# tomer196/GaUDI

Hardware: AMD Instinct MI355X
Metric: guided molecules/sec (1000-step) (higher is better)
Workload: dtype f32

## Files before the change

gaudi_amd/csrc/gaudi_hip.hip:

```cpp
#include <hip/hip_runtime.h>

#include <algorithm>
#include <climits>
#include <queue>
#include <cmath>
#include <cstdio>
#include <cstdlib>
#include <chrono>
#include <cstring>
#include <map>
#include <mutex>
#include <string>
#include <vector>

#include "../../include/gaudi_hip.h"
#include "sampler_kernel.h"

using namespace gaudi;

struct DevBuf {
  void* p = nullptr;
  size_t cap = 0;
  hipError_t reserve(size_t bytes) {
    if (bytes <= cap) return hipSuccess;
// ... 682 lines not shown
#define X(name) kernel_fn gaudi_kern8s_##name(int hpe, int hpp);
GAUDI_KERNEL8S_TUS(X)
#undef X
static kernel_fn pick_kernel8s(int hpe, int hpp) {
  kernel_fn f = nullptr;
#define X(name) \
  if (!f) f = gaudi_kern8s_##name(hpe, hpp);
  GAUDI_KERNEL8S_TUS(X)
#undef X
  return f;
}

#ifdef GAUDI_STAMP_STUBS
#define GAUDI_KERNEL8S2_TUS(X)
#else
#define GAUDI_KERNEL8S2_TUS(X) X(edm_192) X(fused_tiny) X(fused_192_208)
#endif
#define X(name) kernel_fn gaudi_kern8s2_##name(int hpe, int hpp);
GAUDI_KERNEL8S2_TUS(X)
#undef X
static kernel_fn pick_kernel8s2(int hpe, int hpp) {
  kernel_fn f = nullptr;
#define X(name) \
  if (!f) f = gaudi_kern8s2_##name(hpe, hpp);
  GAUDI_KERNEL8S2_TUS(X)
#undef X
  (void)hpe; (void)hpp;
  return f;
}

#ifdef GAUDI_STAMP_STUBS
// ... 93 lines not shown
  size_t net = 0;
  if (hpe)
    net = std::max(net, (size_t)((gn ? 0 : 4 * N * (hpe + 4)) + kWaves * 16 * (hpe + 4) + 8 * N + kWaves * EW * 9 + (6 + ef) * hpe +
                                 (ef > 2 ? kWaves * EW * ef : 0)));
  if (hpp) net = std::max(net, (size_t)((gn ? 0 : 5 * N * (hpp + 4)) + kWaves * 16 * (hpp + 4) + 12 * N + kWaves * EW * 10 + 32 + 10 * hpp));
  return sizeof(float) * (common_floats(N, D, EW) + net);
}
static size_t gnode_floats(int hpe, int hpp, int N) {
  return std::max((size_t)(hpe ? 4 * N * (hpe + 4) : 0), (size_t)(hpp ? 5 * N * (hpp + 4) : 0));
}

static size_t lds_floats8_base(int hpe, int hpp, int N, int D, int S, int split, int gn = 0) {
  size_t net = 0;
  const int pbuf = gn == 3 ? 4 : 5;
  if (gn == 3) gn = 0;
  if (hpe) net = std::max(net, (size_t)((gn ? w8::gn_lds_buffers(gn) : 5) * N * (hpe + 4) + w8::edge_ring_floats(hpe, split) + 8 * N + 2 * align4(N) + 96 + S * 9 + 8 * hpe));
  if (hpp) net = std::max(net, (size_t)(w8::edge_ring_floats(hpp, split) + (gn ? w8::gn_lds_buffers(gn) : pbuf) * N * (hpp + 4) + 12 * N + 2 * align4(N) + 96 + S * 10 + 32 + 10 * hpp));
  return common_floats8(N, D, S) + net;
}
static size_t gnode_floats8(int hpe, int hpp, int N) {
  return std::max((size_t)(hpe ? 5 * N * (hpe + 4) : 0), (size_t)(hpp ? 5 * N * (hpp + 4) : 0));
}
static bool gn8_stage_fits(int hpe, int hpp, int N) {
  for (int hp : {hpe, hpp})
    if (hp && 2 * (size_t)w8::stage_stride(N * (hp + 4)) > w8::edge_ring_floats(hp, 1)) return false;
  return true;
}
static bool node_f16_fits(int hp, int N, int split, bool gn) {
  if (!hp || !split || !GAUDI_NODE_F16) return true;
  if (N > (gn ? 48 : 32)) return false;
  const int nct = N <= 16 ? 1 : N <= 32 ? 2 : 3;
  const int ring = w8::edge_ring_floats(hp, split);
// ... 16 lines not shown
  const int nch = (T + pub_ch - 1) / pub_ch;
  pub_ch = (T + nch - 1) / nch;
  pubx = (int)std::max(0LL, (long long)S * (16 * pub_ch + 4) - own);
  return true;
}
static size_t lds_bytes8(int hpe, int hpp, int N, int D, int S, int pubx, int split, int gn = 0) {
  return sizeof(float) * (lds_floats8_base(hpe, hpp, N, D, S, split, gn) + (hpp ? pubx : 0));
}

static int launch(gaudi_handle* h, const KParams& P, int hpe, int hpp, long long steps) {
  const bool v8 = h->run_variant == 8;
  const bool se = hpe && h->ecfg.sin_embedding;
  kernel_fn fn = v8   ? (h->run_pg && hpe && hpp ? pick_kernel8mp(hpe, hpp) : h->run_gn8 == 2 ? pick_kernel8gp(hpe, hpp) : h->run_gn8 ? pick_kernel8g(hpe, hpp) : pick_kernel8_mode(hpe, hpp, h->run_split, h->run_mr && hpp))
                 : se ? pick_kernel_se(hpe, hpp, h->run_gn)
                      : h->run_gn ? pick_kernel_g(hpe, hpp) : pick_kernel(hpe, hpp);
  if (v8 && !h->run_gn8 && h->run_split == 1 && !(h->run_mr && hpp) && P.N > 16 && !getenv("GAUDI_NO_FR"))
    if (kernel_fn f2 = pick_kernel8s2(hpe, hpp)) fn = f2;
  if (!fn)
    return fail(h, GAUDI_E_INVALID,
                "no kernel instantiated for padded hidden sizes (" + std::to_string(hpe) + "," + std::to_string(hpp) + ")" +
                    (v8 ? " in the 8-wave family" : se ? " among the sin_embedding kernels" : ""));
  size_t lds = v8 ? lds_bytes8(hpe, hpp, P.N, 3 + P.F, P.EW, P.pubx, h->run_split, h->run_pg && hpe && hpp ? 3 : h->run_gn8)
                  : lds_bytes(hpe, hpp, P.N, 3 + P.F, P.EW, h->run_gn, se ? 24 : 2);
  if (v8 && P.hk_off) lds = sizeof(float) * ((size_t)P.hk_off + (size_t)h->run_hk);
  if (lds > 160 * 1024)
    return fail(h, GAUDI_E_CAPACITY, "molecule needs " + std::to_string(lds) + " B of LDS (>160 KiB): N too large");
  {
    static std::mutex attr_mu;
    static std::map<std::pair<int, const void*>, int> granted_by_fn;
    std::lock_guard<std::mutex> lock(attr_mu);
    int& granted = granted_by_fn[{h->device, (const void*)fn}];
    if ((int)lds > granted) {
// ... 1511 lines not shown
```

gaudi_amd/csrc/w8_edm.h:

```cpp
#pragma once
#include "edm_device.h"
#include "w8_common.h"
#include "w8_split.h"
#include "w8_nodes_f16.h"

namespace gaudi {
namespace w8 {

__host__ __device__ constexpr int gn_lds_buffers(int gn) { return gn == 2 ? 2 : 0; }
template <int HP, int SP = 0, int GN = 0>
struct NetSmem {
  static constexpr bool kGlobalNodes = GN != 0;
  float *h, *p, *q;
  float *agg, *agg1;
  float* ring;
  float *x, *x0;
  uint32_t *pmax, *qmax;
  float* hsc;
  f4* geo;
  float* d0;
  float* trans;
  float* vec;
  float* hk = nullptr;
  __host__ __device__ static int floats(int N, int S) {
    return (GN ? gn_lds_buffers(GN) : 5) * N * (HP + 4) + EdgeRing<HP, SP>::kFloats + 8 * N + 2 * align4(N) + 96 + S * 9 + 8 * HP;
  }
  __device__ void carve(float* base, int N, int S, float* gnode = nullptr) {
    constexpr int LD = HP + 4;
    ring = base; base += EdgeRing<HP, SP>::kFloats;
    if (GN) gnode = assume_global(gnode);
    float*& nb = GN ? gnode : base;
    h = nb; nb += N * LD;
    if (GN == 2) {
      p = base; base += N * LD;
      q = base; base += N * LD;
    } else {
      p = nb; nb += N * LD;
      q = nb; nb += N * LD;
    }
    agg = nb; nb += N * LD;
    agg1 = nb; nb += N * LD;
    x = base; base += 4 * N;
    x0 = base; base += 4 * N;
    pmax = (uint32_t*)base; base += align4(N);
    qmax = (uint32_t*)base; base += align4(N);
    hsc = base; base += 96;
    geo = (f4*)base; base += S * 4;
    d0 = base; base += S;
    trans = base; base += S * 4;
    vec = base;
  }
};

template <class SM>
__device__ __forceinline__ void compute_geo(const SM& sm, const MolGraph& mg, float norm_constant, int tid, bool write_d0) {
  for (int slot = tid; slot < mg.ntiles * 16; slot += kThreads) {
    const uint32_t e = mg.edge[slot];
    const int i = ew_i(e), j = ew_j(e);
    const float dx = sm.x[4 * i + 0] - sm.x[4 * j + 0];
    const float dy = sm.x[4 * i + 1] - sm.x[4 * j + 1];
    const float dz = sm.x[4 * i + 2] - sm.x[4 * j + 2];
// ... 97 lines not shown
  float* const xs0 = sm.ring;
  float* const xs1 = sm.ring + stage_stride(N * LD);
  if constexpr (!RI) er_start<HP>(ring, wbe, lay.gcl(0, 0) + 2 * PK, wave, lane);
  typename NodePFSel<HP, NH>::type pf;
  node_prefetch_x<HP, NH, kAheadOne>(pf, wb, wbe, lay.gcl(0, 0), mg.NC, wave, lane, tw);
  auto hctx = [&]() {
    if constexpr (NH) {
      if constexpr (RI) return node_ctx_h<HP>(sm.ring, EdgeRing<HP, SP>::kFloats, mg.NC, W.hinv, tw, sm.hsc);
      else return node_ctx_h<HP>(ring.slot(ring.par ^ 1), EdgeRing<HP, SP>::kFloats / 2, mg.NC, W.hinv, tw, sm.hsc);
    } else {
      return NodeCtxH{1.f, nullptr, nullptr, tw, nullptr};
    }
  };
  const bool keep = NH && sm.hk != nullptr;
  bool h_kept = false;
  constexpr int NV = (7 * HP + 16 + kThreads - 1) / kThreads;
  VecPF<NV> vpf;
  vec_prefetch<NV, kThreads>(vpf, wb, lay.gcl(0, 0) + 6 * PK, 7 * HP + 16, tid);
  STAMP(ST_EDM_IO);

  for (int l = 0; l < W.L; ++l) {
    compute_geo(sm, mg, W.norm_constant, tid, false);
    STAMP(ST_GEO);
    for (int s = 0; s < W.S; ++s) {
      const int G = lay.gcl(l, s);
      const int Wnext_edge = s + 1 < W.S ? lay.gcl(l, s + 1) + 2 * PK : lay.equ(l) + 2 * PK;
      if constexpr (STG) stage_rows(xs0, sm.h, N * LD, wave, lane);
      for (int idx = tid; idx < N * (LD / 4); idx += kThreads) {
        *(f4*)(sm.agg + 4 * idx) = splat(0.f);
        *(f4*)(sm.agg1 + 4 * idx) = splat(0.f);
// ... 41 lines not shown
            const f4 wv = *(const f4*)(wa + 16 * t + 4 * g);
            sdot += m[0] * wv[0] + m[1] * wv[1] + m[2] * wv[2] + m[3] * wv[3];
          }
          float a = 1.f;
          if (W.attention) a = sigmoid_f(reduce_groups(sdot) + ba);
          const float sc = a * tc.mk;
#pragma unroll
          for (int t = 0; t < T; ++t) acc[t] = acc[t] * sc;
          scatter_runs<HP>(acc, tc, sm.agg, sm.agg1, g);
        }
        STAMP(ST_EDGE_EPI);
      }
      __syncthreads();
      STAMP(ST_BARRIER);
      if constexpr (STG) stage_rows(xs0, sm.h, N * LD, wave, lane);
      for (int idx = tid; idx < N * (HP / 4); idx += kThreads) {
        const int n = idx / (HP / 4), f = 4 * (idx % (HP / 4));
        if constexpr (STG)
          *(f4*)(xs1 + n * LD + f) = (*(const f4*)(sm.agg + n * LD + f) + *(const f4*)(sm.agg1 + n * LD + f)) / W.normf;
        else
          *(f4*)(sm.agg + n * LD + f) = (*(const f4*)(sm.agg + n * LD + f) + *(const f4*)(sm.agg1 + n * LD + f)) / W.normf;
      }
      if constexpr (STG) stage_wait();
      else __syncthreads();
      STAMP(ST_MISC);
      node_gemm_x<HP, EPI_SILU, true, GN, NH, kAheadOne, kAheadOne, FL>(wb, wbe, G + 3 * PK, sm.h, xs0, !h_kept, G + 4 * PK, sm.agg, xs1, bn1, sm.p, nullptr, nullptr,
                                              mg.NC, wave, lane, tw, keep ? node_ctx_keep<HP>(hctx(), sm.hk, mg.NC) : hctx(), pf, G + 5 * PK);
      STAMP(ST_NODE);
      __syncthreads();
      STAMP(ST_BARRIER);
      vec_prefetch<NV, kThreads>(vpf, wb, s + 1 < W.S ? lay.gcl(l, s + 1) + 6 * PK : lay.equ(l) + 3 * PK,
                                 s + 1 < W.S ? 7 * HP + 16 : 5 * HP + 16, tid);
      if constexpr (STG) {
        stage_rows(xs0, sm.p, N * LD, wave, lane);
        stage_wait();
      }
      node_gemm_x<HP, EPI_RESIDUAL_MASK, false, GN, NH, kAheadOne, kAheadOne, FL>(wb, wbe, G + 5 * PK, sm.p, xs0, true, -1, nullptr, nullptr, bn2, sm.h, sm.h, mg.mask,
                                                       mg.NC, wave, lane, tw, hctx(), pf,
                                                       s + 1 < W.S ? lay.gcl(l, s + 1) : lay.equ(l));
      h_kept = false;
      STAMP(ST_NODE);
      __syncthreads();
      STAMP(ST_BARRIER);
    }
    {
      const int E = lay.equ(l);
      const int Wnext_edge = l + 1 < W.L ? lay.gcl(l + 1, 0) + 2 * PK : -1;
      vec_commit<NV, kThreads>(vpf, sm.vec, 5 * HP + 16, tid);
      if (tid < N) {
        sm.pmax[tid] = 0u;
        sm.qmax[tid] = 0u;
      }
      if constexpr (STG) {
        stage_rows(xs0, sm.h, N * LD, wave, lane);
        stage_wait();
// ... 107 lines not shown
```

gaudi_amd/csrc/w8_nodes_f16.h:

```cpp
#pragma once
#include "w8_split.h"

namespace gaudi {
namespace w8 {


constexpr float kLoScale = 2048.f;
#ifndef GAUDI_NODE_ABLATE
#define GAUDI_NODE_ABLATE 0
#endif
constexpr int kAblateH = GAUDI_NODE_ABLATE;
#ifndef GAUDI_NODE_STAMPS
#define GAUDI_NODE_STAMPS 0
#endif
#ifndef GAUDI_NODE_PRIO
#define GAUDI_NODE_PRIO 1
#endif
struct NodeStampH {
  unsigned long long sum[8], last;
  __device__ __forceinline__ void start() { last = __builtin_amdgcn_s_memtime(); }
  __device__ __forceinline__ void mark(int i) {
    const unsigned long long t = __builtin_amdgcn_s_memtime();
    sum[i] += t - last;
    last = t;
// ... 48 lines not shown


__host__ __device__ constexpr int nh_bpos(int c, int g) { return (16 * g + (c ^ g)) * 4; }
struct SplitRowH {
  f4 x;
  uint32_t mx;
};
template <int HP>
__device__ __forceinline__ SplitRowH split_row_load(const float* X, int n, int lane) {
  constexpr int LD = HP + 4;
  SplitRowH r;
  r.x = lane < HP / 4 ? *(const f4*)(X + n * LD + 4 * lane) : splat(0.f);
  r.mx = umax(umax(absbits(r.x[0]), absbits(r.x[1])), umax(absbits(r.x[2]), absbits(r.x[3])));
  return r;
}
template <int HP>
__device__ __forceinline__ void split_row_store(const SplitBufH& sb, const f4 x, uint32_t mx, int n, int lane) {
  constexpr int T = HP / 16, nc = nh_chunks(HP);
  const int m = lane >> 3, g = (lane >> 1) & 3, half = lane & 1;
  int k = 141 - (int)(mx >> 23);
  k = k > 126 ? 126 : k;
  const float s = __builtin_bit_cast(float, (uint32_t)(k + 127) << 23), inv = __builtin_bit_cast(float, (uint32_t)(127 - k) << 23);
  const float y0 = x[0] * s, y1 = x[1] * s, y2 = x[2] * s, y3 = x[3] * s;
  const uint32_t h01 = pk_f16(y0, y1), h23 = pk_f16(y2, y3);
  const f2 f01 = unpk_f16(h01), f23 = unpk_f16(h23);
  const uint32_t l01 = pk_f16((y0 - f01[0]) * kLoScale, (y1 - f01[1]) * kLoScale),
                 l23 = pk_f16((y2 - f23[0]) * kLoScale, (y3 - f23[1]) * kLoScale);
  const int ct = n >> 4, c = n & 15;
  if (m < nc) {
    float* d = sb.chunk(m) + ct * 512 + nh_bpos(c, g) + half * 2;
    *(u2*)d = (u2){h01, h23};
    *(u2*)(d + 256) = (u2){l01, l23};
  } else if (nh_odd(HP) && lane < HP / 4) {
    float* d = sb.tail(HP) + ct * 256 + 4 * (lane - 4 * (T - 1)) * 16 + c;
    d[0] = x[0];
    d[16] = x[1];
    d[32] = x[2];
    d[48] = x[3];
  }
  if (lane == 0) sb.scale(HP)[ct * 16 + c] = inv;
}
template <int HP>
__device__ __forceinline__ void split_rows_h(const SplitBufH& sb, const float* X, int N, int wave, int lane) {
  for (int n = wave; n < N; n += 2 * kWaves) {
    const int n2 = n + kWaves < N ? n + kWaves : n;
    SplitRowH a = split_row_load<HP>(X, n, lane), b = split_row_load<HP>(X, n2, lane);
    a.mx = wave_max_u32(a.mx);
// ... 55 lines not shown
  constexpr int nd = AHEAD < NodeGeoH<HP>::D ? AHEAD : NodeGeoH<HP>::D;
  const TileLanesH<HP> tl(wave, lane);
  static_for<nd>([&](auto d_tag) {
    constexpr int d = decltype(d_tag)::value;
    nh_load<HP>(pf.s[d], wh, 2 * W + d * nh_chunk_floats(HP), wave, tl);
  });
}

struct NodeCtxH {
  float winv;
  float* split_a;
  float* split_b;
  bool ktail;
  float* scales;
  float* scales_b = nullptr;
};

template <int HP, int EPI, bool TWO, int MAXNT, int PIN = kAheadOne, int POUT = kAheadOne, bool FL = false>
__device__ __forceinline__ void node_gemm_h(const WBuf& wh, int Wa, const float* sXa, bool do_split_a, int Wb, const float* sXb,
                                            const float* sBias, float* sY, const float* sRes, const float* sMask, int N, int wave,
                                            int lane, const NodeCtxH& cx, NodePFH<HP>& pf, int nextW = -1, float* gPre = nullptr,
                                            uint32_t* sMaxOut = nullptr ,
                                            NodeStampH* ns = nullptr) {
  (void)ns;
  using G = NodeGeoH<HP>;
  constexpr int T = G::T, LD = HP + 4, NTW = G::NTW, nc = G::nc, D = G::D;
  constexpr int kIn = PIN < D ? PIN : D, kOut = POUT < D ? POUT : D;
  constexpr int kLate = nc < D ? 0 : (GAUDI_NODE_LATE < kOut ? GAUDI_NODE_LATE : kOut);
  const int c = lane & 15, g = lane >> 4;
  const int nt = (MAXNT < 2 || N <= 16) ? 1 : (MAXNT < 3 || N <= 32) ? 2 : 3;
  const bool seq = TWO && cx.split_b == cx.split_a;
  const SplitBufH sa{cx.split_a, nt, cx.scales}, sb{cx.split_b, nt, cx.scales_b != nullptr ? cx.scales_b : cx.scales + kScaleFloatsH};
  const int bpos = nh_bpos(c, g);
// ... 10 lines not shown
    for (int u = 0; u < NTW; ++u) {
      const int t = wave + kWaves * u < T ? wave + kWaves * u : 0;
#pragma unroll
      for (int q = 0; q < 4; ++q) {
        const int ln = (q == 0 || !cx.ktail) ? tl.l[u] : kOOBLane;
        ta[u][q] = __builtin_bit_cast(float, __builtin_amdgcn_raw_buffer_load_b32(wh.r, ln * 4, (2 * Wa + nh_tail_off(HP) + t * 256 + q * 64) * 4, 0));
        if constexpr (TWO)
          tb[u][q] = __builtin_bit_cast(float, __builtin_amdgcn_raw_buffer_load_b32(wh.r, ln * 4, (2 * Wb + nh_tail_off(HP) + t * 256 + q * 64) * 4, 0));
      }
    }
  }
  NSTAMP(0);
  if (!(kAblateH & 1)) {
    const int ls = FL ? fresh(lane) : lane;
    if (do_split_a) split_rows_h<HP>(sa, sXa, N, wave, ls);
    if (TWO && !seq) split_rows_h<HP>(sb, sXb, N, wave, ls);
    NSTAMP(1);
    if (do_split_a || (TWO && !seq)) lds_barrier();
    NSTAMP(2);
  }

  f4 acc0[MAXNT][NTW], acc1[MAXNT][NTW], y[MAXNT][NTW];
#pragma unroll
  for (int j = 0; j < MAXNT; ++j)
#pragma unroll
    for (int u = 0; u < NTW; ++u) {
      const int t = wave + kWaves * u < T ? wave + kWaves * u : 0;
      acc0[j][u] = splat(0.f);
      acc1[j][u] = splat(0.f);
      y[j][u] = sBias != nullptr ? *(const f4*)(sBias + 16 * t + 4 * g) : splat(0.f);
    }
  struct BH {
    u4 h, l;
// ... 92 lines not shown
      lds_barrier();
      split_rows_h<HP>(sb, sXb, N, wave, FL ? fresh(lane) : lane);
      lds_barrier();
    }
    source(std::integral_constant<int, 1>{}, sb);
    late(std::integral_constant<int, kOut - kLate>{});
    fold(sb, tb);
  }
  static_for<D>([&](auto d_tag) {
    if constexpr (decltype(d_tag)::value > kOut - kLate) late(d_tag);
  });
#if GAUDI_NODE_PRIO
  if constexpr (!FL) __builtin_amdgcn_s_setprio(0);
#endif
  const int le = FL ? fresh(lane) : lane, ce = le & 15, ge = le >> 4;
  static_for<MAXNT>([&](auto j_tag) {
    constexpr int j = decltype(j_tag)::value;
    if (j < nt) {
#pragma unroll
      for (int u = 0; u < NTW; ++u) {
        const int t = wave + kWaves * u;
        const int nd = j * 16 + ce;
        f4 yy = y[j][u];
        if (t < T && nd < N) {
          float* dst = sY + nd * LD + 16 * t + 4 * ge;
          const bool pad = G::odd && cx.ktail && t == T - 1 && ge > 0;
          if (pad) yy = splat(0.f);
          if (gPre != nullptr) nstash_store((f4*)(gPre + nd * HP + 16 * t + 4 * ge), yy);
          if (sMaxOut != nullptr) atomicMax(sMaxOut + nd, umax(umax(absbits(yy[0]), absbits(yy[1])), umax(absbits(yy[2]), absbits(yy[3]))));
          if (!pad) {
            if (EPI == EPI_SILU) yy = silu4v(yy);
            if (EPI == EPI_RESIDUAL_MASK) {
              const f4 r = *(const f4*)(sRes + nd * LD + 16 * t + 4 * ge);
              yy = (r + yy) * sMask[nd];
            }
            if (EPI == EPI_MUL_DSILU) {
              const f4 r = *(const f4*)(sRes + nd * LD + 16 * t + 4 * ge);
              yy = yy * dsilu4v(r);
            }
            if (EPI == EPI_ACCUM) yy = *(const f4*)(sRes + nd * LD + 16 * t + 4 * ge) + yy;
          }
          *(f4*)dst = yy;
        }
      }
    }
  });
  NSTAMP(6);
}

#ifndef GAUDI_NODE_F16
#define GAUDI_NODE_F16 1
#endif
template <int SP>
struct NodeMath {
  static constexpr bool kF16 = SP != 0 && GAUDI_NODE_F16 != 0;
};
template <int HP, bool NH>
struct NodePFSel {
  using type = NodePF<HP>;
};
template <int HP>
struct NodePFSel<HP, true> {
  using type = NodePFH<HP>;
};
template <int HP, bool NH, int AHEAD, class PF>
__device__ __forceinline__ void node_prefetch_x(PF& pf, const WBuf& wb, const WBuf& wbe, int W, int N, int wave, int lane, bool tw) {
  if constexpr (NH) node_prefetch_h<HP, AHEAD>(pf, wbe, W, wave, lane);
  else node_prefetch<HP>(pf, wb, W, wave, lane, tw);
}
template <int HP, int EPI, bool TWO, int GN, bool NH, int PIN, int POUT, bool FL = false, class PF>
__device__ __forceinline__ void node_gemm_x(const WBuf& wb, const WBuf& wbe, int Wa, const float* Xa, const float* XaS, bool split_a, int Wb,
                                            const float* Xb, const float* XbS, const float* sBias, float* sY, const float* sRes,
                                            const float* sMask, int N, int wave, int lane, bool tw, const NodeCtxH& cx, PF& pf,
                                            int nextW = -1, float* gPre = nullptr, uint32_t* sMaxOut = nullptr) {
  if constexpr (NH) {
    node_gemm_h<HP, EPI, TWO, GN ? 3 : 2, PIN, POUT, FL>(wbe, Wa, Xa, split_a, Wb, Xb, sBias, sY, sRes, sMask, N, wave, lane, cx, pf, nextW, gPre,
                                                         sMaxOut);
  } else if constexpr (GN != 0) {
    node_gemm_n<HP, EPI, true, 3>(wb, Wa, XaS, Wb, XbS, sBias, sY, sRes, sMask, N, wave, lane, tw, &pf, nextW, gPre);
  } else {
    node_gemm<HP, EPI, true>(wb, Wa, Xa, Wb, Xb, sBias, sY, sRes, sMask, N, wave, lane, tw, &pf, nextW, gPre);
  }
}
__host__ __device__ constexpr bool node_ring_idle(int HP, int SP, bool GN) {
  return GN || (SP != 0 && GAUDI_NODE_F16 != 0 && (SP == 2 || HP < 48));
}
template <int HP>
__device__ __forceinline__ NodeCtxH node_ctx_h(float* region, int cap, int N, float winv, bool ktail, float* scales) {
  const int nct = N <= 16 ? 1 : N <= 32 ? 2 : 3;
  const int need = nh_split_floats(HP, nct);
  return NodeCtxH{winv, region, 2 * need <= cap ? region + need : region, ktail, scales};
}
__host__ __device__ constexpr int nh_keep_floats(int HP, int N) { return nh_split_floats(HP, N <= 16 ? 1 : N <= 32 ? 2 : 3) + kScaleFloatsH; }
template <int HP>
__device__ __forceinline__ NodeCtxH node_ctx_keep(const NodeCtxH& cx, float* keep, int N) {
  const int nct = N <= 16 ? 1 : N <= 32 ? 2 : 3;
  return NodeCtxH{cx.winv, keep + kScaleFloatsH, cx.split_a, cx.ktail, keep, cx.scales};
  (void)nct;
}

}
}
```

gaudi_amd/csrc/w8_pred.h:

```cpp
#pragma once
#include "pred_device.h"
#include "w8_edm.h"

namespace gaudi {
namespace w8 {

template <int HP, int SP = 0, int GN = 0, bool PG = false>
struct PredSmem {
  static_assert(!(PG && GN != 0), "PG is a variant of the resident kernels");
  static_assert(!GN || SP != 0, "global node buffers: split edge GEMMs only (the fp32 form's publish buffer starts in b0 / b1)");
  static constexpr bool kGlobalNodes = GN != 0;
  float *b2, *b3, *b4;
  float *b0, *b1;
  float* ring;
  float* pub;
  float *x, *x0, *dx;
  uint32_t *pmax, *qmax;
  float* hsc;
  f4* geo;
  float *d0, *trans, *dd0;
  float* pred;
  float* vec;
  float* hk = nullptr;
  __host__ __device__ static int floats(int N, int S, int pubx) {
    return EdgeRing<HP, SP>::kFloats + (GN ? gn_lds_buffers(GN) : PG ? 4 : 5) * N * (HP + 4) + pubx + 12 * N + 2 * align4(N) + 96 + S * 10 + 32 + 10 * HP;
  }
  __device__ __forceinline__ float* publish() const { return GN ? ring : b0; }
  __device__ void carve(float* base, int N, int S, int pubx, float* gnode = nullptr) {
    constexpr int LD = HP + 4;
    if (SP == 0) { ring = base; base += EdgeRing<HP, SP>::kFloats; }
    if (GN || PG) gnode = assume_global(gnode);
    float*& nb = GN ? gnode : base;
    if (GN == 2) { b2 = base; base += N * LD; } else { b2 = nb; nb += N * LD; }
    b3 = nb; nb += N * LD;
    if (PG) { b4 = gnode; gnode += N * LD; } else { b4 = nb; nb += N * LD; }
    b0 = nb; nb += N * LD;
    if (GN == 2) { b1 = base; base += N * LD; } else { b1 = nb; nb += N * LD; }
    if (SP != 0) { ring = base; base += EdgeRing<HP, SP>::kFloats; }
    pub = base; base += pubx;
    x = base; base += 4 * N;
    x0 = base; base += 4 * N;
    dx = base; base += 4 * N;
    pmax = (uint32_t*)base; base += align4(N);
    qmax = (uint32_t*)base; base += align4(N);
    hsc = base; base += 96;
    geo = (f4*)base; base += S * 4;
    d0 = base; base += S;
    trans = base; base += S * 4;
    dd0 = base; base += S;
    pred = base; base += 32;
    vec = base;
  }
};

__host__ __device__ inline long long pred_stash_floats8(int N, int HP, int L, int S) {
  return pred_stash_node_floats(N, HP, L) + (long long)L * S * HP * 2 + 2LL * L * S + (S > 16 * kWaves ? (long long)S * HP : 0);
}
__device__ __forceinline__ size_t edge_stash_off8(int l, int tile, int arr, int S, int HP) {
  return (((size_t)l * (S / 16) + tile) * 2 + arr) * (size_t)(16 * HP);
}
// ... 47 lines not shown
  constexpr bool STG = GN && !NH;
  float* const xs0 = sm.ring;
  float* const xs1 = sm.ring + stage_stride(N * LD);
  if constexpr (!RI) er_start<HP>(ring, wbe, lay.layer(0) + 2 * HP * HP, wave, lane);
  typename NodePFSel<HP, NH>::type pf;
  node_prefetch_x<HP, NH, kAheadOne>(pf, wb, wbe, lay.layer(0), mg.NC, wave, lane, tw);
  auto hctx = [&]() {
    if constexpr (NH) {
      if constexpr (RI) return node_ctx_h<HP>(sm.ring, EdgeRing<HP, SP>::kFloats, mg.NC, W.hinv, tw, sm.hsc);
      else return node_ctx_h<HP>(ring.slot(ring.par ^ 1), EdgeRing<HP, SP>::kFloats / 2, mg.NC, W.hinv, tw, sm.hsc);
    } else {
      return NodeCtxH{1.f, nullptr, nullptr, tw, nullptr};
    }
  };
  const bool keep = NH && sm.hk != nullptr;
  constexpr int NV = (PredLayerW::vec_count(HP) + kThreads - 1) / kThreads;
  VecPF<NV> vpf;
  vec_prefetch<NV, kThreads>(vpf, wb, PredLayerW::vec_off(lay.layer(0), HP), PredLayerW::vec_count(HP), tid);

  for (int l = 0; l < W.L; ++l) {
    const bool last = l == W.L - 1;
    const PredLayerW Lw(w, lay.layer(l), HP, sm.vec);
    vec_commit<NV, kThreads>(vpf, sm.vec, PredLayerW::vec_count(HP), tid);
    if constexpr (STG) stage_rows(xs0, h, N * LD, wave, lane);
    for (int idx = tid; idx < N * LD; idx += kThreads) {
      agg[idx] = 0.f;
      agg1[idx] = 0.f;
    }
    if (tid < N) {
      sm.pmax[tid] = 0u;
      sm.qmax[tid] = 0u;
    }
    float* st = stash + (size_t)l * (3 * N * HP + 4 * N);
    for (int idx = tid; idx < N; idx += kThreads) gstore4((f4*)(st + 3 * N * HP) + idx, *(const f4*)(sm.x + 4 * idx));
    compute_geo(sm, mg, 1.0f, tid, false);
    if constexpr (STG) stage_wait();
    else __syncthreads();
    STAMP(ST_STAGE);
    {
      const NodeCtxH cx = keep ? node_ctx_keep<HP>(hctx(), sm.hk, mg.NC) : hctx();
      node_gemm_x<HP, EPI_NONE, false, GN, NH, kAheadOne, kAheadAll, FL>(wb, wbe, Lw.A, h, xs0, true, -1, nullptr, nullptr, Lw.b1, p, nullptr, nullptr, mg.NC, wave,
                                                    lane, tw, cx, pf, Lw.Bm, nullptr, sm.pmax);
      node_gemm_x<HP, EPI_NONE, false, GN, NH, kAheadAll, kAheadOne, FL>(wb, wbe, Lw.Bm, h, xs0, false, -1, nullptr, nullptr, nullptr, q, nullptr, nullptr, mg.NC,
                                                    wave, lane, tw, cx, pf, Lw.Wn1h, nullptr, sm.qmax);
    }
    STAMP(ST_NODE);
    __syncthreads();
    STAMP(ST_BARRIER);
    if constexpr (RI) er_start<HP>(ring, wbe, Lw.W2, wave, lane);
    for (int idx = tid; idx < N * (HP / 4); idx += kThreads) {
      const int n = idx / (HP / 4), f = 4 * (idx % (HP / 4));
      nstash_store((f4*)st + idx, *(const f4*)(p + n * LD + f));
      nstash_store((f4*)(st + N * HP) + idx, *(const f4*)(q + n * LD + f));
    }
    STAMP(ST_STASH);
    int rd = 0;
// ... 49 lines not shown
          }
          const float phi = reduce_groups(sdot);
          if (g == 0) gstore(pstash + (size_t)l * S + tc.slot, phi);
          const float tau = (W.use_tanh ? tanhf(phi) * W.coords_range_layer : phi) * tc.mk;
          if (g == 0) *(f4*)(sm.trans + 4 * tc.slot) = (f4){gg[1] * tau, gg[2] * tau, gg[3] * tau, 0.f};
        }
        STAMP(ST_EDGE_EPI);
      }
      if constexpr (MR) {
        if (++rd < mg.rounds) goto pred_fwd_round;
      }
    }
    __syncthreads();
    STAMP(ST_BARRIER);
    if constexpr (STG) stage_rows(xs0, h, N * LD, wave, lane);
    for (int idx = tid; idx < N * (HP / 4); idx += kThreads) {
      const int n = idx / (HP / 4), f = 4 * (idx % (HP / 4));
      if constexpr (STG)
        *(f4*)(xs1 + n * LD + f) = *(const f4*)(agg + n * LD + f) + *(const f4*)(agg1 + n * LD + f);
      else
        *(f4*)(agg + n * LD + f) = *(const f4*)(agg + n * LD + f) + *(const f4*)(agg1 + n * LD + f);
    }
    if constexpr (STG) stage_wait();
    else __syncthreads();
    STAMP(ST_MISC);
    node_gemm_x<HP, EPI_SILU, true, GN, NH, kAheadOne, kAheadOne, FL>(wb, wbe, Lw.Wn1h, h, xs0, !keep, Lw.Wn1a, agg, xs1, Lw.bn1, p, nullptr, nullptr, mg.NC, wave, lane,
                                            tw, keep ? node_ctx_keep<HP>(hctx(), sm.hk, mg.NC) : hctx(), pf, Lw.Wn2, st + 2 * N * HP );
    STAMP(ST_NODE);
    __syncthreads();
    STAMP(ST_BARRIER);
    vec_prefetch<NV, kThreads>(vpf, wb, PredLayerW::vec_off(lay.layer(l + 1 < W.L ? l + 1 : l), HP), PredLayerW::vec_count(HP), tid);
    if constexpr (STG) {
      stage_rows(xs0, p, N * LD, wave, lane);
      stage_wait();
    }
    node_gemm_x<HP, EPI_RESIDUAL_MASK, false, GN, NH, kAheadOne, kAheadOne, FL>(wb, wbe, Lw.Wn2, p, xs0, true, -1, nullptr, nullptr, Lw.bn2, h, h, mg.mask, mg.NC, wave,
                                                     lane, tw, hctx(), pf, l + 1 < W.L ? lay.layer(l + 1) : -1);
    if (!last) coord_update(sm, mg, 1.0f, tid);
    STAMP(ST_NODE);
    __syncthreads();
    STAMP(ST_BARRIER);
  }
  {
    const float* ow = w + lay.out_w();
    const float* ob = w + lay.out_b();
    const float* msk = mg.mask;
    small_dots<kThreads>(
        N * K, HP, tid, [=](int qq, int f) { return gload(ow + (qq % K) * HP + f); },
        [=](int qq, int f) { return h[(qq / K) * LD + f]; },
        [=](int qq, float acc) { p[qq] = (acc + gload(ob + qq % K)) * msk[qq / K]; });
    __syncthreads();
    if (tid < K) {
// ... 39 lines not shown
    __syncthreads();
    compute_geo(sm, mg, 0.f, tid, true);
    __syncthreads();
  }
  {
    const float* ow = w + lay.out_w();
    for (int idx = tid; idx < N * HP; idx += kThreads) {
      const int n = idx / HP, f = idx % HP;
      float acc = 0.f;
      for (int k = 0; k < K; ++k) acc += (dpred[k] / readout_div) * gload(ow + k * HP + f);
      dh[n * LD + f] = acc * mg.mask[n];
    }
    for (int idx = tid; idx < N * 4; idx += kThreads) sm.dx[idx] = 0.f;
    for (int idx = tid; idx < S; idx += kThreads) sm.dd0[idx] = 0.f;
  }
  __syncthreads();

  typename EdgeRing<HP, SP>::type ring;
  er_init<HP>(ring, sm.ring, W.ktail != 0, W.ws, W.hinv);
  constexpr bool NH = NodeMath<SP>::kF16;
  constexpr bool RI = node_ring_idle(HP, SP, GN);
  constexpr bool STG = GN && !NH;
  float* const xs0 = sm.ring;
  float* const xs1 = sm.ring + stage_stride(N * LD);
  if constexpr (!RI) {
    const int L0 = lay.layer(W.L - 1);
    er_start<HP>(ring, wbe, L0 + 9 * HP * HP , wave, lane);
  }
  typename NodePFSel<HP, NH>::type pf;
  node_prefetch_x<HP, NH, kAheadOne>(pf, wb, wbe, lay.layer(W.L - 1) + 13 * HP * HP , mg.NC, wave, lane, tw);
// ... 44 lines not shown
      }
      if (tid < n4) put(tid, p0, q0, v0);
      if (tid + kThreads < n4) put(tid + kThreads, p1, q1, v1);
      for (int idx = tid + 2 * kThreads; idx < n4; idx += kThreads) put(idx, nstash_load(sp + idx), nstash_load(sq + idx), nstash_load(sn + idx));
      for (int idx = tid + kThreads; idx < N; idx += kThreads) {
        *(f4*)(sm.x + 4 * idx) = gload4((const f4*)(st + 3 * N * HP) + idx);
        *(f4*)(sm.dx + 4 * idx) = *(const f4*)(sm.dx + 4 * idx) * mg.mask[idx];
      }
    }
    STAMP(ST_PRED_IO);
    __syncthreads();
    if constexpr (STG) stage_rows(xs0, dh, N * LD, wave, lane);
    compute_geo(sm, mg, 1.0f, tid, false);
    if constexpr (STG) stage_wait();
    STAMP(ST_BWD_EDGE);
    node_gemm_x<HP, EPI_MUL_DSILU, false, GN, NH, kAheadOne, kAheadOne, FL>(wb, wbe, Lw.Wn2t, dh, xs0, true, -1, nullptr, nullptr, nullptr, STG ? xs1 : B4, B4, nullptr,
                                                 mg.NC, wave, lane, tw, hctx(), pf, Lw.Wn1ht);
    __syncthreads();
    {
      const NodeCtxH cx = hctx();
      node_gemm_x<HP, EPI_ACCUM, false, GN, NH, kAheadOne, kAheadAll, FL>(wb, wbe, Lw.Wn1ht, B4, xs1, true, -1, nullptr, nullptr, nullptr, dh, dh, nullptr, mg.NC,
                                                     wave, lane, tw, cx, pf, Lw.Wn1at);
      node_gemm_x<HP, EPI_NONE, false, GN, NH, kAheadAll, 0, FL>(wb, wbe, Lw.Wn1at, B4, xs1, false, -1, nullptr, nullptr, nullptr, B0, nullptr, nullptr,
                                                    mg.NC, wave, lane, tw, cx, pf);
    }
    __syncthreads();
    STAMP(ST_BWD_NODE);
    if constexpr (RI) er_start<HP>(ring, wbe, last ? Lw.W2t : Lw.Wc1t, wave, lane);
    {
      constexpr bool mr = MR;
      int rd = 0;
    pred_bwd_round:
      const bool more = MR && rd + 1 < mg.rounds;
      const TileCols tc = load_tile(mg, MR ? rd : 0, wave, c);
      const int tile = tc.slot >> 4;
      const f4 gg = sm.geo[tc.slot];
// ... 295 lines not shown
```

Baseline: 208.1.

## Produce f16 hi/lo split operands in node GEMM epilogues instead of re-splitting

Result: no change. 209.8, median of 6 (+0.8%).

```diff
diff --git a/gaudi_amd/csrc/gaudi_hip.hip b/gaudi_amd/csrc/gaudi_hip.hip
--- a/gaudi_amd/csrc/gaudi_hip.hip
+++ b/gaudi_amd/csrc/gaudi_hip.hip
@@ -720,7 +720,7 @@
 #ifdef GAUDI_STAMP_STUBS
 #define GAUDI_KERNEL8S2_TUS(X)
 #else
-#define GAUDI_KERNEL8S2_TUS(X) X(edm_192) X(fused_tiny) X(fused_192_208)
+#define GAUDI_KERNEL8S2_TUS(X) X(small) X(edm_192) X(pred_208) X(fused_tiny) X(fused_192_208)
 #endif
 #define X(name) kernel_fn gaudi_kern8s2_##name(int hpe, int hpp);
 GAUDI_KERNEL8S2_TUS(X)
@@ -844,8 +844,8 @@
   size_t net = 0;
   const int pbuf = gn == 3 ? 4 : 5;
   if (gn == 3) gn = 0;
-  if (hpe) net = std::max(net, (size_t)((gn ? w8::gn_lds_buffers(gn) : 5) * N * (hpe + 4) + w8::edge_ring_floats(hpe, split) + 8 * N + 2 * align4(N) + 96 + S * 9 + 8 * hpe));
-  if (hpp) net = std::max(net, (size_t)(w8::edge_ring_floats(hpp, split) + (gn ? w8::gn_lds_buffers(gn) : pbuf) * N * (hpp + 4) + 12 * N + 2 * align4(N) + 96 + S * 10 + 32 + 10 * hpp));
+  if (hpe) net = std::max(net, (size_t)((gn ? w8::gn_lds_buffers(gn) : 5) * N * (hpe + 4) + w8::edge_ring_floats(hpe, split) + 8 * N + 2 * align4(N) + 4 * w8::kScaleFloatsH + S * 9 + 8 * hpe));
+  if (hpp) net = std::max(net, (size_t)(w8::edge_ring_floats(hpp, split) + (gn ? w8::gn_lds_buffers(gn) : pbuf) * N * (hpp + 4) + 12 * N + 2 * align4(N) + 4 * w8::kScaleFloatsH + S * 10 + 32 + 10 * hpp));
   return common_floats8(N, D, S) + net;
 }
 static size_t gnode_floats8(int hpe, int hpp, int N) {
@@ -892,8 +892,13 @@
   kernel_fn fn = v8   ? (h->run_pg && hpe && hpp ? pick_kernel8mp(hpe, hpp) : h->run_gn8 == 2 ? pick_kernel8gp(hpe, hpp) : h->run_gn8 ? pick_kernel8g(hpe, hpp) : pick_kernel8_mode(hpe, hpp, h->run_split, h->run_mr && hpp))
                  : se ? pick_kernel_se(hpe, hpp, h->run_gn)
                       : h->run_gn ? pick_kernel_g(hpe, hpp) : pick_kernel(hpe, hpp);
-  if (v8 && !h->run_gn8 && h->run_split == 1 && !(h->run_mr && hpp) && P.N > 16 && !getenv("GAUDI_NO_FR"))
-    if (kernel_fn f2 = pick_kernel8s2(hpe, hpp)) fn = f2;
+  bool fr = false;
+  if (v8 && !h->run_gn8 && h->run_split == 1 && !(h->run_mr && hpp) && (P.N > 16 || getenv("GAUDI_FORCE_FR")) && !getenv("GAUDI_NO_FR"))
+    if (kernel_fn f2 = pick_kernel8s2(hpe, hpp)) {
+      fn = f2;
+      fr = true;
+    }
+  if (getenv("GAUDI_DEBUG_PLAN")) fprintf(stderr, "[launch] hp=(%d,%d) N=%d fr=%d\n", hpe, hpp, P.N, (int)fr);
   if (!fn)
     return fail(h, GAUDI_E_INVALID,
                 "no kernel instantiated for padded hidden sizes (" + std::to_string(hpe) + "," + std::to_string(hpp) + ")" +
diff --git a/gaudi_amd/csrc/kern8s2_pred_208.hip b/gaudi_amd/csrc/kern8s2_pred_208.hip
--- /dev/null
+++ b/gaudi_amd/csrc/kern8s2_pred_208.hip
@@ -0,0 +1,8 @@
+#include "sampler_kernel.h"
+
+typedef void (*kernel_fn)(const gaudi::KParams);
+
+kernel_fn gaudi_kern8s2_pred_208(int hpe, int hpp) {
+  if (hpe == 0 && hpp == 208) return gaudi::sampler_kernel8s2<0, 208>;
+  return nullptr;
+}
diff --git a/gaudi_amd/csrc/kern8s2_small.hip b/gaudi_amd/csrc/kern8s2_small.hip
--- /dev/null
+++ b/gaudi_amd/csrc/kern8s2_small.hip
@@ -0,0 +1,9 @@
+#include "sampler_kernel.h"
+
+typedef void (*kernel_fn)(const gaudi::KParams);
+
+kernel_fn gaudi_kern8s2_small(int hpe, int hpp) {
+  if (hpe == 32 && hpp == 0) return gaudi::sampler_kernel8s2<32, 0>;
+  if (hpe == 0 && hpp == 48) return gaudi::sampler_kernel8s2<0, 48>;
+  return nullptr;
+}
diff --git a/gaudi_amd/csrc/w8_edm.h b/gaudi_amd/csrc/w8_edm.h
--- a/gaudi_amd/csrc/w8_edm.h
+++ b/gaudi_amd/csrc/w8_edm.h
@@ -23,7 +23,7 @@
   float* vec;
   float* hk = nullptr;
   __host__ __device__ static int floats(int N, int S) {
-    return (GN ? gn_lds_buffers(GN) : 5) * N * (HP + 4) + EdgeRing<HP, SP>::kFloats + 8 * N + 2 * align4(N) + 96 + S * 9 + 8 * HP;
+    return (GN ? gn_lds_buffers(GN) : 5) * N * (HP + 4) + EdgeRing<HP, SP>::kFloats + 8 * N + 2 * align4(N) + 4 * kScaleFloatsH + S * 9 + 8 * HP;
   }
   __device__ void carve(float* base, int N, int S, float* gnode = nullptr) {
     constexpr int LD = HP + 4;
@@ -44,7 +44,7 @@
     x0 = base; base += 4 * N;
     pmax = (uint32_t*)base; base += align4(N);
     qmax = (uint32_t*)base; base += align4(N);
-    hsc = base; base += 96;
+    hsc = base; base += 4 * kScaleFloatsH;
     geo = (f4*)base; base += S * 4;
     d0 = base; base += S;
     trans = base; base += S * 4;
@@ -172,6 +172,9 @@
   };
   const bool keep = NH && sm.hk != nullptr;
   bool h_kept = false;
+  constexpr bool PS = node_produce_split(NH, GN, FL);
+  ProduceMaxH pmx{(uint32_t*)(sm.hsc + 2 * kScaleFloatsH)};
+  if constexpr (PS) pmx.zero(tid);
   constexpr int NV = (7 * HP + 16 + kThreads - 1) / kThreads;
   VecPF<NV> vpf;
   vec_prefetch<NV, kThreads>(vpf, wb, lay.gcl(0, 0) + 6 * PK, 7 * HP + 16, tid);
@@ -243,6 +246,15 @@
       __syncthreads();
       STAMP(ST_BARRIER);
       if constexpr (STG) stage_rows(xs0, sm.h, N * LD, wave, lane);
+      NodeCtxH cx1 = keep ? node_ctx_keep<HP>(hctx(), sm.hk, mg.NC) : hctx();
+      if constexpr (PS && kProduceRowsH) cx1.b_ready = cx1.split_b != cx1.split_a;
+      if (PS && cx1.b_ready) {
+        const float* a0 = sm.agg;
+        const float* a1 = sm.agg1;
+        const float normf = W.normf;
+        produce_rows_h<HP>(pmx.out(cx1, cx1.split_b, cx1.scales_b != nullptr ? cx1.scales_b : cx1.scales + kScaleFloatsH), mg.NC, tid,
+                              [=](int n, int f) { return (*(const f4*)(a0 + n * LD + f) + *(const f4*)(a1 + n * LD + f)) / normf; });
+      } else
       for (int idx = tid; idx < N * (HP / 4); idx += kThreads) {
         const int n = idx / (HP / 4), f = 4 * (idx % (HP / 4));
         if constexpr (STG)
@@ -253,8 +265,12 @@
       if constexpr (STG) stage_wait();
       else __syncthreads();
       STAMP(ST_MISC);
-      node_gemm_x<HP, EPI_SILU, true, GN, NH, kAheadOne, kAheadOne, FL>(wb, wbe, G + 3 * PK, sm.h, xs0, !h_kept, G + 4 * PK, sm.agg, xs1, bn1, sm.p, nullptr, nullptr,
-                                              mg.NC, wave, lane, tw, keep ? node_ctx_keep<HP>(hctx(), sm.hk, mg.NC) : hctx(), pf, G + 5 * PK);
+      {
+        NodeCtxH cx = cx1;
+        if constexpr (PS) cx = pmx.out(cx, hctx().split_a, sm.hsc);
+        node_gemm_x<HP, EPI_SILU, true, GN, NH, kAheadOne, kAheadOne, FL, PS>(wb, wbe, G + 3 * PK, sm.h, xs0, !h_kept, G + 4 * PK, sm.agg, xs1, bn1,
+                                                                             PS ? nullptr : sm.p, nullptr, nullptr, mg.NC, wave, lane, tw, cx, pf, G + 5 * PK);
+      }
       STAMP(ST_NODE);
       __syncthreads();
       STAMP(ST_BARRIER);
@@ -264,10 +280,15 @@
         stage_rows(xs0, sm.p, N * LD, wave, lane);
         stage_wait();
       }
-      node_gemm_x<HP, EPI_RESIDUAL_MASK, false, GN, NH, kAheadOne, kAheadOne, FL>(wb, wbe, G + 5 * PK, sm.p, xs0, true, -1, nullptr, nullptr, bn2, sm.h, sm.h, mg.mask,
-                                                       mg.NC, wave, lane, tw, hctx(), pf,
-                                                       s + 1 < W.S ? lay.gcl(l, s + 1) : lay.equ(l));
-      h_kept = false;
+      {
+        NodeCtxH cx = hctx();
+        if constexpr (PS)
+          if (keep) cx = pmx.out(cx, sm.hk + kScaleFloatsH, sm.hk);
+        node_gemm_x<HP, EPI_RESIDUAL_MASK, false, GN, NH, kAheadOne, kAheadOne, FL, PS>(wb, wbe, G + 5 * PK, sm.p, xs0, !PS, -1, nullptr, nullptr, bn2, sm.h, sm.h,
+                                                                                     mg.mask, mg.NC, wave, lane, tw, cx, pf,
+                                                                                     s + 1 < W.S ? lay.gcl(l, s + 1) : lay.equ(l));
+      }
+      h_kept = PS && keep;
       STAMP(ST_NODE);
       __syncthreads();
       STAMP(ST_BARRIER);
diff --git a/gaudi_amd/csrc/w8_nodes_f16.h b/gaudi_amd/csrc/w8_nodes_f16.h
--- a/gaudi_amd/csrc/w8_nodes_f16.h
+++ b/gaudi_amd/csrc/w8_nodes_f16.h
@@ -86,23 +86,39 @@
   r.mx = umax(umax(absbits(r.x[0]), absbits(r.x[1])), umax(absbits(r.x[2]), absbits(r.x[3])));
   return r;
 }
+struct RowScaleH {
+  float s, inv;
+  __device__ __forceinline__ explicit RowScaleH(uint32_t mx) {
+    int k = 141 - (int)(mx >> 23);
+    k = k > 126 ? 126 : k;
+    s = __builtin_bit_cast(float, (uint32_t)(k + 127) << 23);
+    inv = __builtin_bit_cast(float, (uint32_t)(127 - k) << 23);
+  }
+};
+struct SplitPiecesH {
+  u2 hi, lo;
+  __device__ __forceinline__ SplitPiecesH(const f4 x, float s) {
+    const float y0 = x[0] * s, y1 = x[1] * s, y2 = x[2] * s, y3 = x[3] * s;
+    const uint32_t h01 = pk_f16(y0, y1), h23 = pk_f16(y2, y3);
+    const f2 f01 = unpk_f16(h01), f23 = unpk_f16(h23);
+    const uint32_t l01 = pk_f16((y0 - f01[0]) * kLoScale, (y1 - f01[1]) * kLoScale),
+                   l23 = pk_f16((y2 - f23[0]) * kLoScale, (y3 - f23[1]) * kLoScale);
+    hi = (u2){h01, h23};
+    lo = (u2){l01, l23};
+  }
+};
 template <int HP>
 __device__ __forceinline__ void split_row_store(const SplitBufH& sb, const f4 x, uint32_t mx, int n, int lane) {
   constexpr int T = HP / 16, nc = nh_chunks(HP);
   const int m = lane >> 3, g = (lane >> 1) & 3, half = lane & 1;
-  int k = 141 - (int)(mx >> 23);
-  k = k > 126 ? 126 : k;
-  const float s = __builtin_bit_cast(float, (uint32_t)(k + 127) << 23), inv = __builtin_bit_cast(float, (uint32_t)(127 - k) << 23);
-  const float y0 = x[0] * s, y1 = x[1] * s, y2 = x[2] * s, y3 = x[3] * s;
-  const uint32_t h01 = pk_f16(y0, y1), h23 = pk_f16(y2, y3);
-  const f2 f01 = unpk_f16(h01), f23 = unpk_f16(h23);
-  const uint32_t l01 = pk_f16((y0 - f01[0]) * kLoScale, (y1 - f01[1]) * kLoScale),
-                 l23 = pk_f16((y2 - f23[0]) * kLoScale, (y3 - f23[1]) * kLoScale);
+  const RowScaleH rs(mx);
+  const float inv = rs.inv;
+  const SplitPiecesH pc(x, rs.s);
   const int ct = n >> 4, c = n & 15;
   if (m < nc) {
     float* d = sb.chunk(m) + ct * 512 + nh_bpos(c, g) + half * 2;
-    *(u2*)d = (u2){h01, h23};
-    *(u2*)(d + 256) = (u2){l01, l23};
+    *(u2*)d = pc.hi;
+    *(u2*)(d + 256) = pc.lo;
   } else if (nh_odd(HP) && lane < HP / 4) {
     float* d = sb.tail(HP) + ct * 256 + 4 * (lane - 4 * (T - 1)) * 16 + c;
     d[0] = x[0];
@@ -188,9 +204,29 @@
   bool ktail;
   float* scales;
   float* scales_b = nullptr;
-};
-
-template <int HP, int EPI, bool TWO, int MAXNT, int PIN = kAheadOne, int POUT = kAheadOne, bool FL = false>
+  float* out_split = nullptr;
+  float* out_scales = nullptr;
+  uint32_t* out_max = nullptr;
+  uint32_t* idle_max = nullptr;
+  bool b_ready = false;
+};
+struct ProduceMaxH {
+  uint32_t* base;
+  int par = 0;
+  __device__ __forceinline__ void zero(int tid) const {
+    if (tid < 2 * kScaleFloatsH) base[tid] = 0u;
+  }
+  __device__ __forceinline__ NodeCtxH out(NodeCtxH cx, float* region, float* scales) {
+    cx.out_split = region;
+    cx.out_scales = scales;
+    cx.out_max = base + par * kScaleFloatsH;
+    cx.idle_max = base + (par ^ 1) * kScaleFloatsH;
+    par ^= 1;
+    return cx;
+  }
+};
+
+template <int HP, int EPI, bool TWO, int MAXNT, int PIN = kAheadOne, int POUT = kAheadOne, bool FL = false, bool PS = false>
 __device__ __forceinline__ void node_gemm_h(const WBuf& wh, int Wa, const float* sXa, bool do_split_a, int Wb, const float* sXb,
                                             const float* sBias, float* sY, const float* sRes, const float* sMask, int N, int wave,
                                             int lane, const NodeCtxH& cx, NodePFH<HP>& pf, int nextW = -1, float* gPre = nullptr,
@@ -231,9 +267,10 @@
   if (!(kAblateH & 1)) {
     const int ls = FL ? fresh(lane) : lane;
     if (do_split_a) split_rows_h<HP>(sa, sXa, N, wave, ls);
-    if (TWO && !seq) split_rows_h<HP>(sb, sXb, N, wave, ls);
+    const bool split_b_now = TWO && !seq && !cx.b_ready;
+    if (split_b_now) split_rows_h<HP>(sb, sXb, N, wave, ls);
     NSTAMP(1);
-    if (do_split_a || (TWO && !seq)) lds_barrier();
+    if (do_split_a || split_b_now) lds_barrier();
     NSTAMP(2);
   }
 
@@ -356,6 +393,8 @@
   if constexpr (!FL) __builtin_amdgcn_s_setprio(0);
 #endif
   const int le = FL ? fresh(lane) : lane, ce = le & 15, ge = le >> 4;
+  static_assert(!(PS && FL), "the produce-side split is built for the plain instantiations");
+  const bool prod = PS && cx.out_split != nullptr;
   static_for<MAXNT>([&](auto j_tag) {
     constexpr int j = decltype(j_tag)::value;
     if (j < nt) {
@@ -382,12 +421,93 @@
             }
             if (EPI == EPI_ACCUM) yy = *(const f4*)(sRes + nd * LD + 16 * t + 4 * ge) + yy;
           }
-          *(f4*)dst = yy;
+          if constexpr (PS) {
+            if (prod) {
+              atomicMax(cx.out_max + nd, umax(umax(absbits(yy[0]), absbits(yy[1])), umax(absbits(yy[2]), absbits(yy[3]))));
+              y[j][u] = yy;
+            }
+            if (sY != nullptr) *(f4*)dst = yy;
+          } else {
+            *(f4*)dst = yy;
+          }
         }
       }
     }
   });
-  NSTAMP(6);
+  if constexpr (PS) {
+    if (prod) {
+      lds_barrier();
+      NSTAMP(6);
+      const SplitBufH so{cx.out_split, nt, cx.out_scales};
+      const int lp = fresh(lane), ce = lp & 15, ge = lp >> 4;
+      static_for<MAXNT>([&](auto j_tag) {
+        constexpr int j = decltype(j_tag)::value;
+        const int nd = j * 16 + ce;
+        if (j < nt && nd < N) {
+          const RowScaleH rs(cx.out_max[nd]);
+#pragma unroll
+          for (int u = 0; u < NTW; ++u) {
+            const int t = wave + kWaves * u;
+            if (t < T) {
+              const f4 x = y[j][u];
+              if (G::odd && t == T - 1) {
+                float* d = so.tail(HP) + j * 256 + 4 * ge * 16 + ce;
+                d[0] = x[0];
+                d[16] = x[1];
+                d[32] = x[2];
+                d[48] = x[3];
+              } else {
+                const SplitPiecesH pc(x, rs.s);
+                float* d = so.chunk(t >> 1) + j * 512 + nh_bpos(ce, 2 * (t & 1) + (ge >> 1)) + (ge & 1) * 2;
+                *(u2*)d = pc.hi;
+                *(u2*)(d + 256) = pc.lo;
+              }
+            }
+          }
+          if (wave == 0 && ge == 0) so.scale(HP)[nd] = rs.inv;
+        }
+      });
+      if (wave == 0 && lp < kScaleFloatsH) cx.idle_max[lp] = 0u;
+    }
+  }
+  NSTAMP(PS ? 7 : 6);
+}
+
+template <int HP, class F>
+__device__ __forceinline__ void produce_rows_h(const NodeCtxH& cx, int N, int tid_, F value) {
+  constexpr int Q = HP / 4, T = HP / 16, nc = nh_chunks(HP);
+  const SplitBufH so{cx.out_split, N <= 16 ? 1 : N <= 32 ? 2 : 3, cx.out_scales};
+  {
+    const int tid = fresh(tid_);
+    for (int idx = tid; idx < N * Q; idx += kThreads) {
+      const int n = idx / Q;
+      const f4 v = value(n, 4 * (idx % Q));
+      atomicMax(cx.out_max + n, umax(umax(absbits(v[0]), absbits(v[1])), umax(absbits(v[2]), absbits(v[3]))));
+    }
+  }
+  lds_barrier();
+  {
+    const int tid = fresh(tid_);
+    for (int idx = tid; idx < N * Q; idx += kThreads) {
+      const int n = idx / Q, q = idx % Q, ct = n >> 4, c = n & 15;
+      const f4 v = value(n, 4 * q);
+      const RowScaleH rs(cx.out_max[n]);
+      if ((q >> 3) < nc) {
+        const SplitPiecesH pc(v, rs.s);
+        float* d = so.chunk(q >> 3) + ct * 512 + nh_bpos(c, (q >> 1) & 3) + (q & 1) * 2;
+        *(u2*)d = pc.hi;
+        *(u2*)(d + 256) = pc.lo;
+      } else if (nh_odd(HP)) {
+        float* d = so.tail(HP) + ct * 256 + 4 * (q - 4 * (T - 1)) * 16 + c;
+        d[0] = v[0];
+        d[16] = v[1];
+        d[32] = v[2];
+        d[48] = v[3];
+      }
+      if (q == 0) so.scale(HP)[n] = rs.inv;
+    }
+    if (tid < kScaleFloatsH) cx.idle_max[tid] = 0u;
+  }
 }
 
 #ifndef GAUDI_NODE_F16
@@ -410,13 +530,13 @@
   if constexpr (NH) node_prefetch_h<HP, AHEAD>(pf, wbe, W, wave, lane);
   else node_prefetch<HP>(pf, wb, W, wave, lane, tw);
 }
-template <int HP, int EPI, bool TWO, int GN, bool NH, int PIN, int POUT, bool FL = false, class PF>
+template <int HP, int EPI, bool TWO, int GN, bool NH, int PIN, int POUT, bool FL = false, bool PS = false, class PF>
 __device__ __forceinline__ void node_gemm_x(const WBuf& wb, const WBuf& wbe, int Wa, const float* Xa, const float* XaS, bool split_a, int Wb,
                                             const float* Xb, const float* XbS, const float* sBias, float* sY, const float* sRes,
                                             const float* sMask, int N, int wave, int lane, bool tw, const NodeCtxH& cx, PF& pf,
                                             int nextW = -1, float* gPre = nullptr, uint32_t* sMaxOut = nullptr) {
   if constexpr (NH) {
-    node_gemm_h<HP, EPI, TWO, GN ? 3 : 2, PIN, POUT, FL>(wbe, Wa, Xa, split_a, Wb, Xb, sBias, sY, sRes, sMask, N, wave, lane, cx, pf, nextW, gPre,
+    node_gemm_h<HP, EPI, TWO, GN ? 3 : 2, PIN, POUT, FL, PS>(wbe, Wa, Xa, split_a, Wb, Xb, sBias, sY, sRes, sMask, N, wave, lane, cx, pf, nextW, gPre,
                                                          sMaxOut);
   } else if constexpr (GN != 0) {
     node_gemm_n<HP, EPI, true, 3>(wb, Wa, XaS, Wb, XbS, sBias, sY, sRes, sMask, N, wave, lane, tw, &pf, nextW, gPre);
@@ -433,6 +553,11 @@
   const int need = nh_split_floats(HP, nct);
   return NodeCtxH{winv, region, 2 * need <= cap ? region + need : region, ktail, scales};
 }
+#ifndef GAUDI_NODE_PS
+#define GAUDI_NODE_PS 1
+#endif
+__host__ __device__ constexpr bool node_produce_split(bool NH, int GN, bool FL) { return GAUDI_NODE_PS >= 1 && NH && GN == 0 && !FL; }
+constexpr bool kProduceRowsH = GAUDI_NODE_PS >= 2;
 __host__ __device__ constexpr int nh_keep_floats(int HP, int N) { return nh_split_floats(HP, N <= 16 ? 1 : N <= 32 ? 2 : 3) + kScaleFloatsH; }
 template <int HP>
 __device__ __forceinline__ NodeCtxH node_ctx_keep(const NodeCtxH& cx, float* keep, int N) {
diff --git a/gaudi_amd/csrc/w8_pred.h b/gaudi_amd/csrc/w8_pred.h
--- a/gaudi_amd/csrc/w8_pred.h
+++ b/gaudi_amd/csrc/w8_pred.h
@@ -23,7 +23,7 @@
   float* vec;
   float* hk = nullptr;
   __host__ __device__ static int floats(int N, int S, int pubx) {
-    return EdgeRing<HP, SP>::kFloats + (GN ? gn_lds_buffers(GN) : PG ? 4 : 5) * N * (HP + 4) + pubx + 12 * N + 2 * align4(N) + 96 + S * 10 + 32 + 10 * HP;
+    return EdgeRing<HP, SP>::kFloats + (GN ? gn_lds_buffers(GN) : PG ? 4 : 5) * N * (HP + 4) + pubx + 12 * N + 2 * align4(N) + 4 * kScaleFloatsH + S * 10 + 32 + 10 * HP;
   }
   __device__ __forceinline__ float* publish() const { return GN ? ring : b0; }
   __device__ void carve(float* base, int N, int S, int pubx, float* gnode = nullptr) {
@@ -43,7 +43,7 @@
     dx = base; base += 4 * N;
     pmax = (uint32_t*)base; base += align4(N);
     qmax = (uint32_t*)base; base += align4(N);
-    hsc = base; base += 96;
+    hsc = base; base += 4 * kScaleFloatsH;
     geo = (f4*)base; base += S * 4;
     d0 = base; base += S;
     trans = base; base += S * 4;
@@ -121,6 +121,10 @@
     }
   };
   const bool keep = NH && sm.hk != nullptr;
+  bool h_kept = false;
+  constexpr bool PS = node_produce_split(NH, GN, FL);
+  ProduceMaxH pmx{(uint32_t*)(sm.hsc + 2 * kScaleFloatsH)};
+  if constexpr (PS) pmx.zero(tid);
   constexpr int NV = (PredLayerW::vec_count(HP) + kThreads - 1) / kThreads;
   VecPF<NV> vpf;
   vec_prefetch<NV, kThreads>(vpf, wb, PredLayerW::vec_off(lay.layer(0), HP), PredLayerW::vec_count(HP), tid);
@@ -146,7 +150,7 @@
     STAMP(ST_STAGE);
     {
       const NodeCtxH cx = keep ? node_ctx_keep<HP>(hctx(), sm.hk, mg.NC) : hctx();
-      node_gemm_x<HP, EPI_NONE, false, GN, NH, kAheadOne, kAheadAll, FL>(wb, wbe, Lw.A, h, xs0, true, -1, nullptr, nullptr, Lw.b1, p, nullptr, nullptr, mg.NC, wave,
+      node_gemm_x<HP, EPI_NONE, false, GN, NH, kAheadOne, kAheadAll, FL>(wb, wbe, Lw.A, h, xs0, !h_kept, -1, nullptr, nullptr, Lw.b1, p, nullptr, nullptr, mg.NC, wave,
                                                     lane, tw, cx, pf, Lw.Bm, nullptr, sm.pmax);
       node_gemm_x<HP, EPI_NONE, false, GN, NH, kAheadAll, kAheadOne, FL>(wb, wbe, Lw.Bm, h, xs0, false, -1, nullptr, nullptr, nullptr, q, nullptr, nullptr, mg.NC,
                                                     wave, lane, tw, cx, pf, Lw.Wn1h, nullptr, sm.qmax);
@@ -226,6 +230,14 @@
     __syncthreads();
     STAMP(ST_BARRIER);
     if constexpr (STG) stage_rows(xs0, h, N * LD, wave, lane);
+    NodeCtxH cx1 = keep ? node_ctx_keep<HP>(hctx(), sm.hk, mg.NC) : hctx();
+    if constexpr (PS && kProduceRowsH) cx1.b_ready = cx1.split_b != cx1.split_a;
+    if (PS && cx1.b_ready) {
+      const float* a0 = agg;
+      const float* a1 = agg1;
+      produce_rows_h<HP>(pmx.out(cx1, cx1.split_b, cx1.scales_b != nullptr ? cx1.scales_b : cx1.scales + kScaleFloatsH), mg.NC, tid,
+                            [=](int n, int f) { return *(const f4*)(a0 + n * LD + f) + *(const f4*)(a1 + n * LD + f); });
+    } else
     for (int idx = tid; idx < N * (HP / 4); idx += kThreads) {
       const int n = idx / (HP / 4), f = 4 * (idx % (HP / 4));
       if constexpr (STG)
@@ -236,8 +248,12 @@
     if constexpr (STG) stage_wait();
     else __syncthreads();
     STAMP(ST_MISC);
-    node_gemm_x<HP, EPI_SILU, true, GN, NH, kAheadOne, kAheadOne, FL>(wb, wbe, Lw.Wn1h, h, xs0, !keep, Lw.Wn1a, agg, xs1, Lw.bn1, p, nullptr, nullptr, mg.NC, wave, lane,
-                                            tw, keep ? node_ctx_keep<HP>(hctx(), sm.hk, mg.NC) : hctx(), pf, Lw.Wn2, st + 2 * N * HP );
+    {
+      NodeCtxH cx = cx1;
+      if constexpr (PS) cx = pmx.out(cx, hctx().split_a, sm.hsc);
+      node_gemm_x<HP, EPI_SILU, true, GN, NH, kAheadOne, kAheadOne, FL, PS>(wb, wbe, Lw.Wn1h, h, xs0, !keep, Lw.Wn1a, agg, xs1, Lw.bn1, PS ? nullptr : p, nullptr,
+                                                                           nullptr, mg.NC, wave, lane, tw, cx, pf, Lw.Wn2, st + 2 * N * HP );
+    }
     STAMP(ST_NODE);
     __syncthreads();
     STAMP(ST_BARRIER);
@@ -246,8 +262,14 @@
       stage_rows(xs0, p, N * LD, wave, lane);
       stage_wait();
     }
-    node_gemm_x<HP, EPI_RESIDUAL_MASK, false, GN, NH, kAheadOne, kAheadOne, FL>(wb, wbe, Lw.Wn2, p, xs0, true, -1, nullptr, nullptr, Lw.bn2, h, h, mg.mask, mg.NC, wave,
-                                                     lane, tw, hctx(), pf, l + 1 < W.L ? lay.layer(l + 1) : -1);
+    {
+      NodeCtxH cx = hctx();
+      if constexpr (PS)
+        if (keep) cx = pmx.out(cx, sm.hk + kScaleFloatsH, sm.hk);
+      node_gemm_x<HP, EPI_RESIDUAL_MASK, false, GN, NH, kAheadOne, kAheadOne, FL, PS>(wb, wbe, Lw.Wn2, p, xs0, !PS, -1, nullptr, nullptr, Lw.bn2, h, h, mg.mask,
+                                                                                   mg.NC, wave, lane, tw, cx, pf, l + 1 < W.L ? lay.layer(l + 1) : -1);
+      h_kept = PS && keep;
+    }
     if (!last) coord_update(sm, mg, 1.0f, tid);
     STAMP(ST_NODE);
     __syncthreads();
@@ -317,6 +339,9 @@
     for (int idx = tid; idx < N * 4; idx += kThreads) sm.dx[idx] = 0.f;
     for (int idx = tid; idx < S; idx += kThreads) sm.dd0[idx] = 0.f;
   }
+  constexpr bool PS = node_produce_split(NodeMath<SP>::kF16, GN, FL);
+  ProduceMaxH pmx{(uint32_t*)(sm.hsc + 2 * kScaleFloatsH)};
+  if constexpr (PS) pmx.zero(tid);
   __syncthreads();
 
   typename EdgeRing<HP, SP>::type ring;
@@ -391,12 +416,16 @@
     compute_geo(sm, mg, 1.0f, tid, false);
     if constexpr (STG) stage_wait();
     STAMP(ST_BWD_EDGE);
-    node_gemm_x<HP, EPI_MUL_DSILU, false, GN, NH, kAheadOne, kAheadOne, FL>(wb, wbe, Lw.Wn2t, dh, xs0, true, -1, nullptr, nullptr, nullptr, STG ? xs1 : B4, B4, nullptr,
-                                                 mg.NC, wave, lane, tw, hctx(), pf, Lw.Wn1ht);
+    {
+      NodeCtxH cx = hctx();
+      if constexpr (PS) cx = pmx.out(cx, cx.split_a, sm.hsc);
+      node_gemm_x<HP, EPI_MUL_DSILU, false, GN, NH, kAheadOne, kAheadOne, FL, PS>(wb, wbe, Lw.Wn2t, dh, xs0, true, -1, nullptr, nullptr, nullptr,
+                                                                                 PS ? nullptr : (STG ? xs1 : B4), B4, nullptr, mg.NC, wave, lane, tw, cx, pf, Lw.Wn1ht);
+    }
     __syncthreads();
     {
       const NodeCtxH cx = hctx();
-      node_gemm_x<HP, EPI_ACCUM, false, GN, NH, kAheadOne, kAheadAll, FL>(wb, wbe, Lw.Wn1ht, B4, xs1, true, -1, nullptr, nullptr, nullptr, dh, dh, nullptr, mg.NC,
+      node_gemm_x<HP, EPI_ACCUM, false, GN, NH, kAheadOne, kAheadAll, FL>(wb, wbe, Lw.Wn1ht, B4, xs1, !PS, -1, nullptr, nullptr, nullptr, dh, dh, nullptr, mg.NC,
                                                      wave, lane, tw, cx, pf, Lw.Wn1at);
       node_gemm_x<HP, EPI_NONE, false, GN, NH, kAheadAll, 0, FL>(wb, wbe, Lw.Wn1at, B4, xs1, false, -1, nullptr, nullptr, nullptr, B0, nullptr, nullptr,
                                                     mg.NC, wave, lane, tw, cx, pf);
```
